# DeepMed-Lab-ECNU/BCP

Hardware: AMD Instinct MI355X
Metric: training volumes/sec (LA 112x112x80 V-Net, BCP self-training step) (higher is better)
Workload: dtype f32 (fp16x2 split operands); 1 GPU; LA 3D V-Net BCP self-train step, per-GPU batch 4 (2 labeled), 112x112x80 patches, SGD m0.9 wd1e-4, EMA 0.99 (BASELINE.json configs[1]); global_batch=4, parallelism=dp1

## Files before the change

### bcp_amd/csrc/api.hip

```cpp
#include "common.h"
#include "../../include/bcp_hip.h"
#include <cstring>

namespace bcp {
static thread_local char g_err[512] = "";
void set_error(const char* fmt, ...) {
  va_list ap;
  va_start(ap, fmt);
  vsnprintf(g_err, sizeof(g_err), fmt, ap);
  va_end(ap);
}
Options& options() {
  static Options o;
  return o;
}
}

extern "C" int bcp_version(void) { return BCP_ABI_VERSION; }

extern "C" int bcp_set_option(const char* name, const char* value) {
  BCP_REQUIRE(name && value, "bcp_set_option: null argument");
  bcp::Options& o = bcp::options();
  const bcp::Options def;
  long long v[5] = {0, 0, 0, 0, 0};
  const int n = sscanf(value, "%lld,%lld,%lld,%lld,%lld", &v[0], &v[1], &v[2], &v[3], &v[4]);
  const bool reset = n <= 0;
#define BCP_OPT_INT(field) if (!strcmp(name, #field)) { o.field = reset ? def.field : (int)v[0]; return BCP_OK; }
  BCP_OPT_INT(conv3_p) BCP_OPT_INT(splitk) BCP_OPT_INT(conv3_b6_flat_sk) BCP_OPT_INT(conv3_b6_cfg2d) BCP_OPT_INT(conv3_b6_w22) BCP_OPT_INT(conv3_b6_pipe) BCP_OPT_INT(conv3_b6_cin16max) BCP_OPT_INT(res_pcu) BCP_OPT_INT(res_nt) BCP_OPT_INT(wgrad_nt)
  BCP_OPT_INT(tn_groups) BCP_OPT_INT(cc_tile) BCP_OPT_INT(pack_sections) BCP_OPT_INT(cc_select_blocks) BCP_OPT_INT(conv3_b6) BCP_OPT_INT(conv3_b6_levels) BCP_OPT_INT(conv3_b6_direct) BCP_OPT_INT(conv3_b6_flat) BCP_OPT_INT(conv3_b6_minvox) BCP_OPT_INT(wgrad_b6) BCP_OPT_INT(wgrad_b6_minvox) BCP_OPT_INT(wgrad_b6_levels) BCP_OPT_INT(wgrad_b6_slots) BCP_OPT_INT(cc_border_dedupe) BCP_OPT_INT(cc_count_tile) BCP_OPT_INT(cc_fuse_select) BCP_OPT_INT(gemm_walk) BCP_OPT_INT(gemm_pipe) BCP_OPT_INT(gemm_stat_r) BCP_OPT_INT(norm_apply_cap) BCP_OPT_INT(norm_apply_vec) BCP_OPT_INT(k2_stats) BCP_OPT_INT(k2_bwd_stats) BCP_OPT_INT(up_recompute) BCP_OPT_INT(wgrad_b6_deep) BCP_OPT_INT(wgrad_b6_deep_nt) BCP_OPT_INT(wgrad_b6_deep_slots) BCP_OPT_INT(wgrad_b6_deep_tile) BCP_OPT_INT(norm_slabs) BCP_OPT_INT(conv3_f16) BCP_OPT_INT(fuse_bwd_stats) BCP_OPT_INT(conv3_xcd) BCP_OPT_INT(mix_c1) BCP_OPT_INT(whatif) BCP_OPT_INT(c3d16_form) BCP_OPT_INT(norm_own) BCP_OPT_INT(wgrad_reduce_flat) BCP_OPT_INT(norm_fin_rows) BCP_OPT_INT(norm_fuse_fin)
#undef BCP_OPT_INT
  if (!strcmp(name, "conv3_sk_elems")) { o.conv3_sk_elems = reset ? def.conv3_sk_elems : v[0]; return BCP_OK; }
  if (!strcmp(name, "res_tile2d_vox")) { o.res_tile2d_vox = reset ? def.res_tile2d_vox : v[0]; return BCP_OK; }
  if (!strcmp(name, "conv3_cfg")) {
    BCP_REQUIRE(reset || n == 4, "bcp_set_option: conv3_cfg wants TD,TH,TW,NT");
    for (int i = 0; i < 4; ++i) o.conv3_cfg[i] = reset ? 0 : (int)v[i];
    return BCP_OK;
  }
  if (!strcmp(name, "wgrad_tile")) {
    BCP_REQUIRE(reset || n >= 3, "bcp_set_option: wgrad_tile wants TD,TH,TW[,min_voxels,max_voxels]");
    for (int i = 0; i < 5; ++i) o.wgrad_tile[i] = def.wgrad_tile[i];
    for (int i = 0; i < n && !reset; ++i) o.wgrad_tile[i] = v[i];
    return BCP_OK;
  }
  bcp::set_error("bcp_set_option: unknown option '%s'", name);
  return BCP_EINVAL;
}
extern "C" const char* bcp_last_error(void) { return bcp::g_err; }

extern "C" int bcp_device_arch(char* buf, int n) {
  BCP_REQUIRE(buf && n > 0, "bcp_device_arch: bad buffer");
  int dev = 0;
  hipDeviceProp_t prop;
  if (hipGetDevice(&dev) != hipSuccess || hipGetDeviceProperties(&prop, dev) != hipSuccess) {
    bcp::set_error("bcp_device_arch: no HIP device");
    return BCP_ELAUNCH;
  }
  strncpy(buf, prop.gcnArchName, (size_t)n - 1);
  buf[n - 1] = 0;
  return BCP_OK;
}

extern "C" int bcp_event_create(void** ev) {
  BCP_REQUIRE(ev, "bcp_event_create: null");
  hipEvent_t e;
  if (hipEventCreate(&e) != hipSuccess) { bcp::set_error("hipEventCreate failed"); return BCP_ELAUNCH; }
  *ev = (void*)e;
  return BCP_OK;
}
extern "C" int bcp_event_record(void* ev, void* stream) {
  if (hipEventRecord((hipEvent_t)ev, (hipStream_t)stream) != hipSuccess) { bcp::set_error("hipEventRecord failed"); return BCP_ELAUNCH; }
  return BCP_OK;
}
extern "C" int bcp_event_elapsed_ms(void* start, void* stop, float* ms) {
  BCP_REQUIRE(ms, "bcp_event_elapsed_ms: null");
  if (hipEventSynchronize((hipEvent_t)stop) != hipSuccess || hipEventElapsedTime(ms, (hipEvent_t)start, (hipEvent_t)stop) != hipSuccess) {
    bcp::set_error("hipEventElapsedTime failed");
    return BCP_ELAUNCH;
  }
  return BCP_OK;
}
extern "C" int bcp_event_destroy(void* ev) {
  hipEventDestroy((hipEvent_t)ev);
// ... 36 lines not shown
```

### bcp_amd/csrc/common.h

```cpp
#pragma once
#include <hip/hip_runtime.h>
#include <cstdarg>
#include <cstdint>
#include <cstdio>

#define BCP_OK 0
#define BCP_EINVAL (-1)
#define BCP_ELAUNCH (-2)
#define BCP_EUNSUP (-3)

typedef float f32x4 __attribute__((ext_vector_type(4)));

namespace bcp {

void set_error(const char* fmt, ...);

#define BCP_REQUIRE(cond, ...)          \
  do {                                  \
    if (!(cond)) {                      \
      ::bcp::set_error(__VA_ARGS__);    \
      return BCP_EINVAL;                \
    }                                   \
  } while (0)

// ... 8 lines not shown

struct Options {
  int conv3_p = 0;
  int splitk = 0;
  long long conv3_sk_elems = 1LL << 20;
  int conv3_b6_cin16max = 32;
  int conv3_b6_pipe = 1;
  int conv3_b6_w22 = 1;
  int conv3_b6_cfg2d = 1;
  int conv3_b6_flat_sk = 0;
  int res_pcu = 0;
  int res_nt = 0;
  long long res_tile2d_vox = 10000;
  int conv3_cfg[4] = {0, 0, 0, 0};
  int wgrad_nt = 0;
  long long wgrad_tile[5] = {0, 0, 0, 0, 1LL << 60};
  int tn_groups = 0;
  int pack_sections = 7;
  int cc_tile = 0;
  int cc_select_blocks = 0;
  int conv3_b6 = 1;
  int conv3_b6_levels = 15;
  int conv3_b6_minvox = 256;
  int conv3_b6_flat = 1;
  int conv3_b6_direct = 1;
  int wgrad_b6 = 1;
  int wgrad_b6_minvox = 256;
  int norm_slabs = 1;
  int fuse_bwd_stats = 1;
  int conv3_xcd = 11;
  int conv3_f16 = 1;
  int wgrad_b6_slots = 0;
  int mix_c1 = 1;
  int wgrad_b6_deep = 1;
  int wgrad_b6_deep_nt = 0;
  int wgrad_b6_deep_slots = 0;
  int wgrad_b6_deep_tile = 1;
  int k2_stats = 2;
  int up_recompute = 0;
  int k2_bwd_stats = 0;
  int norm_fuse_fin = 1;
  int norm_fin_rows = 128;
  int gemm_pipe = 1;
  int gemm_stat_r = 0;
  int gemm_walk = 0;
  int cc_border_dedupe = 1;
  int cc_count_tile = 0;
  int cc_fuse_select = 1;
  int norm_apply_cap = 2048;
  int norm_apply_vec = 4;
  int wgrad_reduce_flat = 1;
  int norm_own = 0;
  int c3d16_form = 1;
  int whatif = 0;
  int wgrad_b6_levels = 15;
};
Options& options();

__device__ __forceinline__ unsigned char plabel_bin_of(float x0, float x1, float thres) {
  const float m = fmaxf(x0, x1);
  const float e0 = expf(x0 - m), e1 = expf(x1 - m);
  const float p1 = e1 / (e0 + e1);
  return (p1 >= thres) ? 1 : 0;
}
__device__ __forceinline__ unsigned char plabel_argmax4_of(float x0, float x1, float x2, float x3) {
  const float m = fmaxf(fmaxf(x0, x1), fmaxf(x2, x3));
  const float e0 = expf(x0 - m), e1 = expf(x1 - m), e2 = expf(x2 - m), e3 = expf(x3 - m);
  const float s = e0 + e1 + e2 + e3;
  const float p0 = e0 / s, p1 = e1 / s, p2 = e2 / s, p3 = e3 / s;
  int best = 0;
  float pb = p0;
  if (p1 > pb) { pb = p1; best = 1; }
  if (p2 > pb) { pb = p2; best = 2; }
  if (p3 > pb) { pb = p3; best = 3; }
  return (unsigned char)best;
}


static inline int cdiv(long long a, long long b) { return (int)((a + b - 1) / b); }
static inline bool aligned16(const void* p) { return (reinterpret_cast<uintptr_t>(p) & 15u) == 0; }

#ifndef BCP_LDS_BARRIER
#define BCP_LDS_BARRIER() asm volatile("s_waitcnt lgkmcnt(0)\n\ts_barrier" ::: "memory")
#endif

#ifndef BCP_GLDS16
typedef __attribute__((address_space(3))) void* bcp_lds_ptr_t;
#define BCP_GLDS16(gsrc, lds_wave_base) __builtin_amdgcn_global_load_lds((gsrc), (bcp_lds_ptr_t)(lds_wave_base), 16, 0, 0)
#define BCP_VM_LDS_BARRIER(N) asm volatile("s_waitcnt vmcnt(%0) lgkmcnt(0)\n\ts_barrier" ::"n"(N) : "memory")
#endif

#ifndef BCP_S_SLEEP
#define BCP_S_SLEEP(n) __builtin_amdgcn_s_sleep(n)
#endif

__device__ __forceinline__ float wave_sum(float v) {
#pragma unroll
  for (int o = 32; o > 0; o >>= 1) v += __shfl_xor(v, o);
  return v;
}
__device__ __forceinline__ double wave_sum(double v) {
#pragma unroll
  for (int o = 32; o > 0; o >>= 1) v += __shfl_xor(v, o);
  return v;
}

__device__ __forceinline__ unsigned long long wave_sum(unsigned long long v) {
#pragma unroll
  for (int o = 32; o > 0; o >>= 1) v += __shfl_xor(v, o);
  return v;
}

template <int NV>
__device__ __forceinline__ void block_sum_256(double (&v)[NV], double* lds ) {
  const int lane = threadIdx.x & 63, wid = threadIdx.x >> 6;
#pragma unroll
  for (int i = 0; i < NV; ++i) v[i] = wave_sum(v[i]);
  __syncthreads();
  if (lane == 0) {
#pragma unroll
    for (int i = 0; i < NV; ++i) lds[wid * NV + i] = v[i];
  }
  __syncthreads();
  if (threadIdx.x == 0) {
#pragma unroll
    for (int i = 0; i < NV; ++i) v[i] = lds[i] + lds[NV + i] + lds[2 * NV + i] + lds[3 * NV + i];
  }
}

constexpr int kAmaxSlots = 32, kAmaxStride = 32, kAmaxFloats = kAmaxSlots * kAmaxStride;
__device__ __forceinline__ void amax_clear(float* __restrict__ slots) {
  if (threadIdx.x < kAmaxSlots) slots[threadIdx.x * kAmaxStride] = 0.f;
}
__device__ __forceinline__ void block_amax_publish(float m, float* __restrict__ slots) {
  __shared__ float amax_red[4];
#pragma unroll
  for (int o = 32; o > 0; o >>= 1) { const float t = __shfl_xor(m, o); m = (t > m || t != t) ? t : m; }
  if ((threadIdx.x & 63) == 0) amax_red[threadIdx.x >> 6] = m;
// ... 46 lines not shown
```

### bcp_amd/csrc/conv3.hip

```cpp
#include "conv3_defs.h"
#include "../../include/bcp_hip.h"
#include <cstdlib>
#include <cstdio>

namespace bcp {

template <int KD, int TD, int TH, int TW, int NT, int WT>
__global__ __launch_bounds__(256) void k_conv3_mfma(const float* __restrict__ X, const float* __restrict__ Wp,
                                                    const float* __restrict__ bias, float* __restrict__ Y, ConvDims cd,
                                                    int accumulate, StatsArg st) {
  using TL = Tile<KD, TD, TH, TW>;
  constexpr int MT = TL::MT, T = TL::T, CT = NT * 16;
  constexpr int S = T / WT;
  static_assert(T % WT == 0, "WT must divide the tap count");
  constexpr int NBUF = (S > 1) ? 2 : 1;
  constexpr int WSTAGE4 = WT * 4 * CT;
  constexpr int NW4 = (WSTAGE4 + 255) / 256;
  constexpr int NACC = (MT * NT == 1) ? 2 : 1;

  HIP_DYNAMIC_SHARED(float4, smem4)
  float* smem = reinterpret_cast<float*>(smem4);
  float* Xs = smem;
  float* Ws = smem + TL::HV * XS;
  double* Ss = reinterpret_cast<double*>(Ws + NBUF * WSTAGE4 * 4);

  const int lane = threadIdx.x & 63, wave = threadIdx.x >> 6;
  const int li = lane & 15, lg = lane >> 4;
  int n, d0, h0, w0;
  tile_origin(cd, blockIdx.x, TD, TH, TW, n, d0, h0, w0);
  const int cout0 = blockIdx.y * CT;
  const int cin4 = cd.Cin16 >> 2;

  int voff[MT];
#pragma unroll
  for (int mt = 0; mt < MT; ++mt) voff[mt] = TL::voff((wave * MT + mt) * 16 + li) * XS + lg * 4;
  HaloFetch<TL> hf;
  hf.init(cd, Xs);

  f32x4 acc[NACC][MT][NT];
#pragma unroll
  for (int a = 0; a < NACC; ++a)
#pragma unroll
    for (int mt = 0; mt < MT; ++mt)
#pragma unroll
      for (int nt = 0; nt < NT; ++nt) acc[a][mt][nt] = (f32x4){0.f, 0.f, 0.f, 0.f};

  const int nchunks = cd.Cin16 >> 4;
  const int c_begin = (int)((long long)nchunks * blockIdx.z / gridDim.z), c_end = (int)((long long)nchunks * (blockIdx.z + 1) / gridDim.z);
  Y += (long long)blockIdx.z * cd.N * cd.D * cd.H * cd.W * cd.Cout;
  if (S == 1) {
    float4 hpre[HaloFetch<TL>::NP], wpre[NW4];
    auto wfetch = [&](int cc) {
#pragma unroll
      for (int u = 0; u < NW4; ++u) {
        const int q = threadIdx.x + u * 256;
// ... 917 lines not shown
      uchar4 m4 = make_uchar4(1, 1, 1, 1);
      if (EPI >= 3 && ok) dav = ld4(nm.da + e);
      if (has_mask && ok) m4 = nm.mask_seed ? bern_keep4(e, mseed_lo, mseed_hi, nm.p_keep) : *reinterpret_cast<const uchar4*>(nm.elem_mask + e);
      f32x4 acc = (f32x4){0.f, 0.f, 0.f, 0.f};
#pragma unroll
      for (int ks = 0; ks < KS; ++ks) acc = __builtin_amdgcn_mfma_f32_16x16x4f32(wv[ks], Xs[vo + toff[ks]], acc, 0, 0, 0);
      float4 dyl = make_float4(0.f, 0.f, 0.f, 0.f);
      if (ok) {
        const float yv[4] = {acc[0] + bv.x, acc[1] + bv.y, acc[2] + bv.z, acc[3] + bv.w};
        if (EPI == 0) st4(Y + e, make_float4(yv[0], yv[1], yv[2], yv[3]));
        if (EPI <= 1) {
          if (st.partial) {
#pragma unroll
            for (int r = 0; r < 4; ++r) { s1[r] += (double)yv[r]; s2[r] += (double)yv[r] * (double)yv[r]; }
          }
        } else {
          const float ms[4] = {m4.x ? nm.elem_scale : 0.f, m4.y ? nm.elem_scale : 0.f, m4.z ? nm.elem_scale : 0.f, m4.w ? nm.elem_scale : 0.f};
          const float dd[4] = {dav.x, dav.y, dav.z, dav.w};
          float o[4];
#pragma unroll
          for (int r = 0; r < 4; ++r) {
            const float z = (yv[r] - mu[r]) * sc[r] + sh[r];
            if (EPI == 2) {
              o[r] = act_fwd(z, nm.act);
              if (has_mask) o[r] *= ms[r];
              const float t = fabsf(o[r]);
              amax_o = (t > amax_o || t != t) ? t : amax_o;
            } else {
              const float cs = has_mask ? ms[r] : 1.f;
              const float dz = dd[r] * cs * act_grad(z, nm.act);
              const float xh = (yv[r] - mu[r]) * rs[r];
              if (EPI == 3) { s1[r] += (double)dz; s2[r] += (double)dz * (double)xh; }
              else o[r] = sc[r] * (dz - k1[r] - xh * k2[r]);
            }
          }
          if (EPI == 2 || EPI == 4) st4(Y + e, make_float4(o[0], o[1], o[2], o[3]));
          if (EPI == 5) dyl = make_float4(o[0], o[1], o[2], o[3]);
        }
      }
      if (EPI == 5) st4(Ys + m * 16 + lg * 4, dyl);
    }
    if (EPI == 5) {
      __syncthreads();
#pragma unroll 4
      for (int ks = 0; ks < 16; ++ks) {
        const int v = wave * 64 + ks * 4 + lg;
        const int vo = TL::voff(v);
        const float b = Ys[v * 16 + li];
        wacc[0] = __builtin_amdgcn_mfma_f32_16x16x4f32(Xs[vo + aoff[0]], b, wacc[0], 0, 0, 0);
        wacc[1] = __builtin_amdgcn_mfma_f32_16x16x4f32(Xs[vo + aoff[1]], b, wacc[1], 0, 0, 0);
      }
    }
  }
  if (EPI == 5) {
    __syncthreads();
    float* red = Ys;
#pragma unroll
    for (int tt = 0; tt < 2; ++tt)
#pragma unroll
      for (int r = 0; r < 4; ++r) red[(wave * 32 + tt * 16 + lg * 4 + r) * 16 + li] = wacc[tt][r];
    __syncthreads();
    for (int o = threadIdx.x; o < T * 16; o += 256)
      Y[(long long)blockIdx.x * T * 16 + o] = (red[o] + red[512 + o]) + (red[1024 + o] + red[1536 + o]);
  }
  if (st.partial) {
#pragma unroll
    for (int r = 0; r < 4; ++r) {
      double a = s1[r], b = s2[r];
#pragma unroll
      for (int o = 1; o < 16; o <<= 1) { a += __shfl_xor(a, o); b += __shfl_xor(b, o); }
      if (li == 0) { Ss[(wave * 16 + lg * 4 + r) * 2] = a; Ss[(wave * 16 + lg * 4 + r) * 2 + 1] = b; }
    }
    __syncthreads();
    if (threadIdx.x < 16) {
      const int c = threadIdx.x;
      double a = 0.0, b = 0.0;
#pragma unroll
      for (int wv_ = 0; wv_ < 4; ++wv_) { a += Ss[(wv_ * 16 + c) * 2]; b += Ss[(wv_ * 16 + c) * 2 + 1]; }
      const int gg = t_begin / st.tiles_per_group, row = (t_begin % st.tiles_per_group) / tiles_per_block;
      double* dst = st.partial + (((long long)gg * st.rows + row) * 16 + c) * 2;
      dst[0] = a; dst[1] = b;
    }
  }
  if (EPI == 2 && nm.amax) { __syncthreads(); block_amax_publish(amax_o, nm.amax); }
}

template <int KD, int TD, int TH, int TW>
__global__ __launch_bounds__(256) void k_conv3_c1_wgrad(const float* __restrict__ X, const float* __restrict__ dY,
                                                        float* __restrict__ partial, ConvDims cd, int tiles_total,
                                                        int tiles_per_group) {
  using TL = Tile<KD, TD, TH, TW>;
  constexpr int T = TL::T, M = TL::M;
  static_assert(M == 256 && T <= 32, "four waves x 64 voxels, two 16-tap MFMA row tiles");
  constexpr int NXS = (TL::HV + 255) / 256;
  __shared__ __attribute__((aligned(16))) float Xs[TL::HV];
  __shared__ __attribute__((aligned(16))) float Ys[M * 16];
  const int lane = threadIdx.x & 63, wave = threadIdx.x >> 6;
  const int li = lane & 15, lg = lane >> 4;
  const int grp = blockIdx.x;
  int t_end = (grp + 1) * tiles_per_group;
  if (t_end > tiles_total) t_end = tiles_total;
  int tile = grp * tiles_per_group;
  if (tile >= t_end) return;

  int aoff[2];
#pragma unroll
// ... 484 lines not shown
  const Cfg c = choose_wgrad_cfg(KD, N, D, H, W, Co16);
  const int g = wgrad_groups(c, N, D, H, W, Ci16, Co16);
  const size_t a = (size_t)g * KD * 9 * Ci16 * Co16 * sizeof(float), c6 = b6_wgrad_workspace_bytes(cd, KD);
  return a > c6 ? a : c6;
}

#define BCP_WG_CASE(KD_, TD_, TH_, TW_, NT_)                                                     \
  if (c.KD == KD_ && c.TD == TD_ && c.TH == TH_ && c.TW == TW_ && c.NT == NT_) {                 \
    G = launch_wgrad<KD_, TD_, TH_, TW_, NT_>(x, dy, ws, cd, groups, (hipStream_t)stream);       \
    done = true;                                                                                 \
  }

extern "C" int bcp_conv3_wgrad(const float* x, const float* dy, float* dw, int N, int D, int H, int W, int Cin, int Cout, int KD,
                               int accumulate, void* workspace, const float* x_amax_or_null, const float* dy_amax_or_null, void* stream) {
  if (bcp::options().whatif & 8) return BCP_OK;

  BCP_REQUIRE(x && dy && dw && workspace, "bcp_conv3_wgrad: null pointer");
  BCP_REQUIRE((KD == 1 || KD == 3) && N > 0 && D > 0 && H > 0 && W > 0, "bcp_conv3_wgrad: bad extents");
  BCP_REQUIRE(Cin % 4 == 0 && Cout % 4 == 0, "bcp_conv3_wgrad: Cin/Cout must be multiples of 4");
  ConvDims cd;
  fill_dims(cd, N, D, H, W, Cin, Cout);
  bool done = false;
  const Cfg c = choose_wgrad_cfg(KD, N, D, H, W, cd.Cout16);
  const int groups = wgrad_groups(c, N, D, H, W, cd.Cin16, cd.Cout16);
  float* ws = reinterpret_cast<float*>(workspace);
  if (x_amax_or_null && dy_amax_or_null) { cd.xamax = x_amax_or_null; cd.yamax = dy_amax_or_null; }
  int G = b6_wgrad(x, dy, ws, dw, accumulate, cd, KD, (hipStream_t)stream);
  if (G < 0) {
    BCP_CHECK_LAUNCH("bcp_conv3_wgrad");
    return BCP_OK;
  }
  if (G > 0) done = true;
  if (!done) {
  BCP_WG_CASE(3, 4, 4, 16, 1) BCP_WG_CASE(3, 4, 4, 16, 2) BCP_WG_CASE(3, 4, 4, 16, 4)
  BCP_WG_CASE(3, 4, 8, 8, 1) BCP_WG_CASE(3, 4, 8, 8, 2) BCP_WG_CASE(3, 4, 8, 8, 4)
  BCP_WG_CASE(3, 4, 4, 8, 1) BCP_WG_CASE(3, 4, 4, 8, 2) BCP_WG_CASE(3, 4, 4, 8, 4)
  BCP_WG_CASE(3, 4, 4, 4, 1) BCP_WG_CASE(3, 4, 4, 4, 2) BCP_WG_CASE(3, 4, 4, 4, 4)
  BCP_WG_CASE(3, 2, 8, 4, 1) BCP_WG_CASE(3, 2, 8, 4, 2) BCP_WG_CASE(3, 2, 8, 4, 4)
  BCP_WG_CASE(1, 1, 16, 16, 1) BCP_WG_CASE(1, 1, 16, 16, 2) BCP_WG_CASE(1, 1, 16, 16, 4)
  BCP_WG_CASE(1, 1, 8, 8, 1) BCP_WG_CASE(1, 1, 8, 8, 2) BCP_WG_CASE(1, 1, 8, 8, 4)
  }
  BCP_REQUIRE(done, "bcp_conv3_wgrad: no kernel instance for KD=%d tile=%dx%dx%d NT=%d", c.KD, c.TD, c.TH, c.TW, c.NT);
  const int T = KD * 9;
  if (G >= 32 || options().wgrad_reduce_flat == 2)
    launch_reduce_deep(ws, dw, G, T, Cin, Cout, cd.Cin16, cd.Cout16, accumulate, (hipStream_t)stream);
  else
    hipLaunchKernelGGL(k_wgrad_reduce, dim3(Cin, cdiv(Cout, 64)), dim3(256), 0, (hipStream_t)stream, ws, dw, G, T, Cin, Cout, cd.Cin16,
                       cd.Cout16, accumulate);
  BCP_CHECK_LAUNCH("bcp_conv3_wgrad");
  return BCP_OK;
}

static int c1_tiles_per_block(int tiles_per_group) {
  for (int t = 8; t > 1; t >>= 1)
    if (tiles_per_group % t == 0 && tiles_per_group / t >= 256) return t;
  return 1;
}

template <int EPI>
static void c1_launch(int KD, dim3 grid, hipStream_t s, const float* x, const float* w, const float* bias, float* y, const ConvDims& cd, int tiles,
                      int tpb, const StatsArg& st, const C1Norm& nm) {
  if (KD == 3) hipLaunchKernelGGL((k_conv3_c1<3, 4, 4, 16, EPI>), grid, dim3(256), 0, s, x, w, bias, y, cd, tiles, tpb, st, nm);
  else hipLaunchKernelGGL((k_conv3_c1<1, 1, 16, 16, EPI>), grid, dim3(256), 0, s, x, w, bias, y, cd, tiles, tpb, st, nm);
}

static int c1_fwd_impl(const float* x, const float* w, const float* bias, float* y, int N, int D, int H, int W, int KD, double* stat_partial,
                       int groups, bool dry, hipStream_t s, int epi = 0, const C1Norm* nmp = nullptr) {
  ConvDims cd;
  fill_dims(cd, N, D, H, W, 1, 16);
  if (KD == 3) { cd.tiles_d = cdiv(D, 4); cd.tiles_h = cdiv(H, 4); cd.tiles_w = cdiv(W, 16); }
  else { cd.tiles_d = 1; cd.tiles_h = cdiv(H, 16); cd.tiles_w = cdiv(W, 16); }
  const int tiles = N * cd.tiles_d * cd.tiles_h * cd.tiles_w;
  StatsArg st{nullptr, 0, 1, 16, groups > 0 ? groups : 1};
  int tpb = 1;
  if (groups > 0) {
    if (N % groups) return 0;
    const int tpg = tiles / groups;
    tpb = c1_tiles_per_block(tpg);
    st.tiles_per_group = tpg; st.rows = tpg / tpb; st.partial = stat_partial;
    if (dry) return st.rows;
  }
  const dim3 grid(cdiv(tiles, tpb));
  const C1Norm none{nullptr, nullptr, nullptr, nullptr, 1.f, 0, 1, nullptr};
  const C1Norm& nm = nmp ? *nmp : none;
  switch (epi) {
    case 1: c1_launch<1>(KD, grid, s, x, w, bias, y, cd, tiles, tpb, st, nm); break;
    case 2: c1_launch<2>(KD, grid, s, x, w, bias, y, cd, tiles, tpb, st, nm); break;
    case 3: c1_launch<3>(KD, grid, s, x, w, bias, y, cd, tiles, tpb, st, nm); break;
    case 4: c1_launch<4>(KD, grid, s, x, w, bias, y, cd, tiles, tpb, st, nm); break;
    case 5: c1_launch<5>(KD, grid, s, x, w, bias, y, cd, tiles, tpb, st, nm); break;
    default: c1_launch<0>(KD, grid, s, x, w, bias, y, cd, tiles, tpb, st, nm); break;
  }
  return st.rows;
}

extern "C" int bcp_conv3_c1_fwd(const float* x, const float* w, const float* bias, float* y, int N, int D, int H, int W, int KD,
                                void* stream) {
  BCP_REQUIRE(x && w && y, "bcp_conv3_c1_fwd: null pointer");
  BCP_REQUIRE((KD == 1 && D == 1) || KD == 3, "bcp_conv3_c1_fwd: bad KD/D");
  BCP_REQUIRE(aligned16(y) && (!bias || aligned16(bias)), "bcp_conv3_c1_fwd: y / bias must be 16-B aligned");
  c1_fwd_impl(x, w, bias, y, N, D, H, W, KD, nullptr, 0, false, (hipStream_t)stream);
  BCP_CHECK_LAUNCH("bcp_conv3_c1_fwd");
  return BCP_OK;
}

extern "C" int bcp_conv3_c1_stat_rows(int N, int D, int H, int W, int KD, int groups) {
  if (groups < 1 || N < 1 || D < 1 || H < 1 || W < 1 || !((KD == 1 && D == 1) || KD == 3)) return 0;
  return c1_fwd_impl(nullptr, nullptr, nullptr, nullptr, N, D, H, W, KD, nullptr, groups, true, nullptr);
}

extern "C" int bcp_conv3_c1_fwd_stats(const float* x, const float* w, const float* bias, float* y, int N, int D, int H, int W, int KD,
                                      double* stat_partial, int groups, void* stream) {
  BCP_REQUIRE(x && w && y && stat_partial && groups >= 1, "bcp_conv3_c1_fwd_stats: null pointer / bad groups");
  BCP_REQUIRE((KD == 1 && D == 1) || KD == 3, "bcp_conv3_c1_fwd_stats: bad KD/D");
  BCP_REQUIRE(aligned16(y) && (!bias || aligned16(bias)), "bcp_conv3_c1_fwd_stats: y / bias must be 16-B aligned");
  const int rows = c1_fwd_impl(x, w, bias, y, N, D, H, W, KD, stat_partial, groups, false, (hipStream_t)stream);
  BCP_REQUIRE(rows > 0, "bcp_conv3_c1_fwd_stats: fused statistics unavailable (N %% groups != 0): check bcp_conv3_c1_stat_rows first");
  BCP_CHECK_LAUNCH("bcp_conv3_c1_fwd_stats");
  return BCP_OK;
}

namespace bcp {
void norm_fwd_finalize_launch(const double* partial, int nb, int G, int C, long long rows_per_group, const float* gamma, const float* beta,
                              float* running_mean, float* running_var, float momentum, float eps, float* stats, hipStream_t s, float* amax_clear_or_null);
void norm_bwd_finalize_launch(const double* partial, int nb, int G, int C, long long rows_per_group, float* dgamma, float* dbeta, int accumulate,
                              float* c1c2raw, hipStream_t s, float* amax_clear_or_null);
}

extern "C" size_t bcp_conv3_c1_norm_workspace_bytes(int N, int D, int H, int W, int KD, int groups) {
  const int rows = bcp_conv3_c1_stat_rows(N, D, H, W, KD, groups);
  return rows > 0 ? (size_t)groups * rows * 16 * 2 * sizeof(double) + (size_t)4 * groups * 16 * sizeof(float) : 0;
}

// ... 103 lines not shown
```

Baseline: 825.0 volumes/s.

## Add streamlined single-input-channel conv kernel with prefetched halo and packed tap offsets

Adds a new k_conv3_c1s kernel for the Cin=1 convolution and selects it by default for KD=3 through the c1_form option. It prefetches the next tile's halo into registers while the MFMAs run on the current one, using double-buffered LDS. Tap offsets are packed into registers and bounds checks are done with one-hot masks. A compile-time all-full variant drops per-tile bounds checks and requests higher occupancy, and sched_group_barrier hints interleave LDS reads with MFMAs. This adds code size and register pressure and depends on correct halo masking at borders; a c1_tpb override is also added.

```diff
diff --git a/bcp_amd/csrc/api.hip b/bcp_amd/csrc/api.hip
--- a/bcp_amd/csrc/api.hip
+++ b/bcp_amd/csrc/api.hip
@@ -27,7 +27,7 @@
   const bool reset = n <= 0;
 #define BCP_OPT_INT(field) if (!strcmp(name, #field)) { o.field = reset ? def.field : (int)v[0]; return BCP_OK; }
   BCP_OPT_INT(conv3_p) BCP_OPT_INT(splitk) BCP_OPT_INT(conv3_b6_flat_sk) BCP_OPT_INT(conv3_b6_cfg2d) BCP_OPT_INT(conv3_b6_w22) BCP_OPT_INT(conv3_b6_pipe) BCP_OPT_INT(conv3_b6_cin16max) BCP_OPT_INT(res_pcu) BCP_OPT_INT(res_nt) BCP_OPT_INT(wgrad_nt)
-  BCP_OPT_INT(tn_groups) BCP_OPT_INT(cc_tile) BCP_OPT_INT(pack_sections) BCP_OPT_INT(cc_select_blocks) BCP_OPT_INT(conv3_b6) BCP_OPT_INT(conv3_b6_levels) BCP_OPT_INT(conv3_b6_direct) BCP_OPT_INT(conv3_b6_flat) BCP_OPT_INT(conv3_b6_minvox) BCP_OPT_INT(wgrad_b6) BCP_OPT_INT(wgrad_b6_minvox) BCP_OPT_INT(wgrad_b6_levels) BCP_OPT_INT(wgrad_b6_slots) BCP_OPT_INT(cc_border_dedupe) BCP_OPT_INT(cc_count_tile) BCP_OPT_INT(cc_fuse_select) BCP_OPT_INT(gemm_walk) BCP_OPT_INT(gemm_pipe) BCP_OPT_INT(gemm_stat_r) BCP_OPT_INT(norm_apply_cap) BCP_OPT_INT(norm_apply_vec) BCP_OPT_INT(k2_stats) BCP_OPT_INT(k2_bwd_stats) BCP_OPT_INT(up_recompute) BCP_OPT_INT(wgrad_b6_deep) BCP_OPT_INT(wgrad_b6_deep_nt) BCP_OPT_INT(wgrad_b6_deep_slots) BCP_OPT_INT(wgrad_b6_deep_tile) BCP_OPT_INT(norm_slabs) BCP_OPT_INT(conv3_f16) BCP_OPT_INT(fuse_bwd_stats) BCP_OPT_INT(conv3_xcd) BCP_OPT_INT(mix_c1) BCP_OPT_INT(whatif) BCP_OPT_INT(c3d16_form) BCP_OPT_INT(norm_own) BCP_OPT_INT(wgrad_reduce_flat) BCP_OPT_INT(norm_fin_rows) BCP_OPT_INT(norm_fuse_fin)
+  BCP_OPT_INT(tn_groups) BCP_OPT_INT(cc_tile) BCP_OPT_INT(pack_sections) BCP_OPT_INT(cc_select_blocks) BCP_OPT_INT(conv3_b6) BCP_OPT_INT(conv3_b6_levels) BCP_OPT_INT(conv3_b6_direct) BCP_OPT_INT(conv3_b6_flat) BCP_OPT_INT(conv3_b6_minvox) BCP_OPT_INT(wgrad_b6) BCP_OPT_INT(wgrad_b6_minvox) BCP_OPT_INT(wgrad_b6_levels) BCP_OPT_INT(wgrad_b6_slots) BCP_OPT_INT(cc_border_dedupe) BCP_OPT_INT(cc_count_tile) BCP_OPT_INT(cc_fuse_select) BCP_OPT_INT(gemm_walk) BCP_OPT_INT(gemm_pipe) BCP_OPT_INT(gemm_stat_r) BCP_OPT_INT(norm_apply_cap) BCP_OPT_INT(norm_apply_vec) BCP_OPT_INT(k2_stats) BCP_OPT_INT(k2_bwd_stats) BCP_OPT_INT(up_recompute) BCP_OPT_INT(wgrad_b6_deep) BCP_OPT_INT(wgrad_b6_deep_nt) BCP_OPT_INT(wgrad_b6_deep_slots) BCP_OPT_INT(wgrad_b6_deep_tile) BCP_OPT_INT(norm_slabs) BCP_OPT_INT(conv3_f16) BCP_OPT_INT(fuse_bwd_stats) BCP_OPT_INT(conv3_xcd) BCP_OPT_INT(mix_c1) BCP_OPT_INT(whatif) BCP_OPT_INT(c3d16_form) BCP_OPT_INT(c1_form) BCP_OPT_INT(c1_tpb) BCP_OPT_INT(norm_own) BCP_OPT_INT(wgrad_reduce_flat) BCP_OPT_INT(norm_fin_rows) BCP_OPT_INT(norm_fuse_fin)
 #undef BCP_OPT_INT
   if (!strcmp(name, "conv3_sk_elems")) { o.conv3_sk_elems = reset ? def.conv3_sk_elems : v[0]; return BCP_OK; }
   if (!strcmp(name, "res_tile2d_vox")) { o.res_tile2d_vox = reset ? def.res_tile2d_vox : v[0]; return BCP_OK; }
diff --git a/bcp_amd/csrc/common.h b/bcp_amd/csrc/common.h
--- a/bcp_amd/csrc/common.h
+++ b/bcp_amd/csrc/common.h
@@ -84,6 +84,8 @@
   int wgrad_reduce_flat = 1;
   int norm_own = 0;
   int c3d16_form = 1;
+  int c1_form = 1;
+  int c1_tpb = 0;
   int whatif = 0;
   int wgrad_b6_levels = 15;
 };
@@ -116,6 +118,18 @@
 #define BCP_LDS_BARRIER() asm volatile("s_waitcnt lgkmcnt(0)\n\ts_barrier" ::: "memory")
 #endif
 
+#ifndef BCP_SETTLE
+#define BCP_SETTLE(x) asm volatile("" : "+v"(x))
+#endif
+
+#ifndef BCP_GLOBAL
+#define BCP_GLOBAL __attribute__((address_space(1)))
+#endif
+
+#ifndef BCP_SCHED_GROUP
+#define BCP_SCHED_GROUP(mask, n) __builtin_amdgcn_sched_group_barrier((mask), (n), 0)
+#endif
+
 #ifndef BCP_GLDS16
 typedef __attribute__((address_space(3))) void* bcp_lds_ptr_t;
 #define BCP_GLDS16(gsrc, lds_wave_base) __builtin_amdgcn_global_load_lds((gsrc), (bcp_lds_ptr_t)(lds_wave_base), 16, 0, 0)
diff --git a/bcp_amd/csrc/conv3.hip b/bcp_amd/csrc/conv3.hip
--- a/bcp_amd/csrc/conv3.hip
+++ b/bcp_amd/csrc/conv3.hip
@@ -1,6 +1,7 @@
 #include "conv3_defs.h"
 #include "../../include/bcp_hip.h"
 #include <cstdlib>
+#include <type_traits>
 #include <cstdio>
 
 namespace bcp {
@@ -1024,6 +1025,346 @@
       }
     }
   }
+  if (EPI == 5) {
+    __syncthreads();
+    float* red = Ys;
+#pragma unroll
+    for (int tt = 0; tt < 2; ++tt)
+#pragma unroll
+      for (int r = 0; r < 4; ++r) red[(wave * 32 + tt * 16 + lg * 4 + r) * 16 + li] = wacc[tt][r];
+    __syncthreads();
+    for (int o = threadIdx.x; o < T * 16; o += 256)
+      Y[(long long)blockIdx.x * T * 16 + o] = (red[o] + red[512 + o]) + (red[1024 + o] + red[1536 + o]);
+  }
+  if (st.partial) {
+#pragma unroll
+    for (int r = 0; r < 4; ++r) {
+      double a = s1[r], b = s2[r];
+#pragma unroll
+      for (int o = 1; o < 16; o <<= 1) { a += __shfl_xor(a, o); b += __shfl_xor(b, o); }
+      if (li == 0) { Ss[(wave * 16 + lg * 4 + r) * 2] = a; Ss[(wave * 16 + lg * 4 + r) * 2 + 1] = b; }
+    }
+    __syncthreads();
+    if (threadIdx.x < 16) {
+      const int c = threadIdx.x;
+      double a = 0.0, b = 0.0;
+#pragma unroll
+      for (int wv_ = 0; wv_ < 4; ++wv_) { a += Ss[(wv_ * 16 + c) * 2]; b += Ss[(wv_ * 16 + c) * 2 + 1]; }
+      const int gg = t_begin / st.tiles_per_group, row = (t_begin % st.tiles_per_group) / tiles_per_block;
+      double* dst = st.partial + (((long long)gg * st.rows + row) * 16 + c) * 2;
+      dst[0] = a; dst[1] = b;
+    }
+  }
+  if (EPI == 2 && nm.amax) { __syncthreads(); block_amax_publish(amax_o, nm.amax); }
+}
+
+template <bool B> struct C1Flag { static constexpr bool value = B; };
+
+template <int KD, int TD, int TH, int TW, int EPI, bool ALL_FULL>
+__global__ __launch_bounds__(256, ALL_FULL ? 4 : 2) void k_conv3_c1s(const float* __restrict__ X, const float* __restrict__ w ,
+                                                                      const float* __restrict__ bias, float* __restrict__ Y, ConvDims cd,
+                                                                      int n_tiles, int tiles_per_block, StatsArg st, C1Norm nm) {
+  constexpr bool all_full = ALL_FULL;
+  using TL = Tile<KD, TD, TH, TW>;
+  constexpr int T = TL::T, MT = TL::MT, KS = (T + 3) / 4;
+  constexpr int HVA = (TL::HV + 3) & ~3;
+  constexpr int AHEAD = KS < 2 ? KS : 2;
+  static_assert(TW == 16 && MT == 4 && TL::M == 256 && TH % MT == 0,
+                "a wave's m-tile is one 16-voxel w line: m = (wave * 4 + mt) * 16 + li, and its four lines are consecutive h");
+  __shared__ __attribute__((aligned(16))) float Xs[2 * HVA];
+  __shared__ float Ws[KS * 64];
+  __shared__ __attribute__((aligned(16))) float Cs[4 * 7 * 4];
+  __shared__ double Ss[4 * 16 * 2];
+  __shared__ __attribute__((aligned(16))) float Ys[EPI == 5 ? TL::M * 16 : 4];
+  static_assert(EPI != 5 || T <= 32, "EPI 5: two 16-tap MFMA row tiles");
+  const int lane = threadIdx.x & 63, wave = threadIdx.x >> 6;
+  const int li = lane & 15, lg = lane >> 4;
+  static_assert(TL::HV <= 1024, "packed tap offsets");
+  unsigned aq = 0;
+  f32x4 wacc[2] = {(f32x4){0.f, 0.f, 0.f, 0.f}, (f32x4){0.f, 0.f, 0.f, 0.f}};
+  if (EPI == 5) {
+#pragma unroll
+    for (int tt = 0; tt < 2; ++tt) aq |= (unsigned)((tt * 16 + li < T) ? TL::tapoff(tt * 16 + li) : 0) << (16 * tt);
+  }
+  unsigned tq[(KS + 2) / 3];
+#pragma unroll
+  for (int j = 0; j < (KS + 2) / 3; ++j) tq[j] = 0;
+#pragma unroll
+  for (int ks = 0; ks < KS; ++ks) {
+    const int tap = ks * 4 + lg;
+    tq[ks / 3] |= (unsigned)(tap < T ? TL::tapoff(tap) : 0) << (10 * (ks % 3));
+    if (wave == 0) Ws[ks * 64 + lane] = tap < T ? w[li * T + tap] : 0.f;
+  }
+  double s1[4] = {0, 0, 0, 0}, s2[4] = {0, 0, 0, 0};
+  float amax_o = 0.f;
+  unsigned mseed_lo = 0, mseed_hi = 0;
+  if (EPI >= 2 && nm.mask_seed) { const unsigned long long s_ = *nm.mask_seed; mseed_lo = (unsigned)s_; mseed_hi = (unsigned)(s_ >> 32); }
+  const bool has_mask = EPI >= 2 && (nm.elem_mask != nullptr || nm.mask_seed != nullptr);
+  const bool a_relu = nm.act == ACT_RELU, a_lrelu = nm.act == ACT_LRELU;
+  const float g_neg = a_lrelu ? 0.01f : (a_relu ? 0.f : 1.f);
+  auto actf = [&](float z) __attribute__((always_inline)) -> float { const float neg = a_lrelu ? 0.01f * z : (a_relu ? 0.f : z); return z > 0.f ? z : neg; };
+  auto actg = [&](float z) __attribute__((always_inline)) -> float { return z > 0.f ? 1.f : g_neg; };
+  const bool mask_ld = EPI >= 2 && nm.elem_mask != nullptr && nm.mask_seed == nullptr;
+  const int t_begin = blockIdx.x * tiles_per_block;
+  int t_end = t_begin + tiles_per_block;
+  if (t_end > n_tiles) t_end = n_tiles;
+  if (wave == 0 && li == 0) {
+    float* c = Cs + lg * 28;
+    st4(c, bias ? ld4(bias + lg * 4) : make_float4(0.f, 0.f, 0.f, 0.f));
+    if (EPI >= 2) {
+      const int g = t_begin / st.tiles_per_group;
+      const long long GC = (long long)nm.G * 16, o = (long long)g * 16 + lg * 4;
+#pragma unroll
+      for (int r = 0; r < 4; ++r) {
+        c[4 + r] = nm.stats[o + r]; c[8 + r] = nm.stats[GC + o + r]; c[12 + r] = nm.stats[2 * GC + o + r]; c[16 + r] = nm.stats[3 * GC + o + r];
+        if (EPI >= 4) { c[20 + r] = nm.c1c2[o + r]; c[24 + r] = nm.c1c2[GC + o + r]; }
+      }
+    }
+  }
+  int tn, ttd, tth, ttw;
+  {
+    int d0, h0, w0;
+    tile_origin(cd, t_begin, TD, TH, TW, tn, d0, h0, w0);
+    tn = __builtin_amdgcn_readfirstlane(tn); ttd = __builtin_amdgcn_readfirstlane(d0 / TD);
+    tth = __builtin_amdgcn_readfirstlane(h0 / TH); ttw = __builtin_amdgcn_readfirstlane(w0 / TW);
+  }
+  auto step = [&]() __attribute__((always_inline)) {
+    ttw += 1;
+    const int cw = ttw == cd.tiles_w ? 1 : 0;
+    ttw = cw ? 0 : ttw; tth += cw;
+    const int ch = tth == cd.tiles_h ? 1 : 0;
+    tth = ch ? 0 : tth; ttd += ch;
+    const int cdd = ttd == cd.tiles_d ? 1 : 0;
+    ttd = cdd ? 0 : ttd; tn += cdd;
+  };
+  constexpr int NPRE = (TL::HV + 255) / 256;
+  constexpr int HB_D = TL::PD ? TL::HD : 0, HBITS = HB_D + TL::HH + TL::HW;
+  static_assert(HBITS <= 64, "one-hot halo coordinates");
+  using hmask_t = typename std::conditional<(HBITS <= 32), unsigned, unsigned long long>::type;
+  float pre[NPRE];
+  unsigned pre_in = 0;
+  unsigned hrel[NPRE];
+  hmask_t hbit[NPRE];
+#pragma unroll
+  for (int i = 0; i < NPRE; ++i) {
+    int q = threadIdx.x + i * 256;
+    if (q > TL::HV - 1) q = TL::HV - 1;
+    const int hw = q % TL::HW, hh = (q / TL::HW) % TL::HH, hd = q / (TL::HW * TL::HH);
+    hrel[i] = (unsigned)((hd * cd.H + hh) * cd.W + hw) * 4u;
+    hbit[i] = ((hmask_t)1 << (HB_D + hh)) | ((hmask_t)1 << (HB_D + TL::HH + hw)) | (TL::PD ? ((hmask_t)1 << hd) : (hmask_t)0);
+  }
+  const unsigned crel = (unsigned)((TL::PD * cd.H + 1) * cd.W + 1) * 4u;
+  auto ival = [](int lo, int hi) __attribute__((always_inline)) -> hmask_t {
+    return (((hmask_t)1 << hi) - 1) & ~(((hmask_t)1 << lo) - 1);
+  };
+  auto fetch = [&](int n, int d0, int h0, int w0) __attribute__((always_inline)) {
+    const long long corner = (((long long)n * cd.D + (d0 - TL::PD)) * cd.H + (h0 - 1)) * cd.W + (w0 - 1);
+    const char* xc = reinterpret_cast<const char*>(X + corner);
+    const int dlo = TL::PD - d0 > 0 ? TL::PD - d0 : 0, dhi = cd.D - d0 + TL::PD < TL::HD ? cd.D - d0 + TL::PD : TL::HD;
+    const int hlo = 1 - h0 > 0 ? 1 - h0 : 0, hhi = cd.H - h0 + 1 < TL::HH ? cd.H - h0 + 1 : TL::HH;
+    const int wlo = 1 - w0 > 0 ? 1 - w0 : 0, whi = cd.W - w0 + 1 < TL::HW ? cd.W - w0 + 1 : TL::HW;
+    const hmask_t tm = (TL::PD ? ival(dlo, dhi) : (hmask_t)0) | (ival(hlo, hhi) << HB_D) | (ival(wlo, whi) << (HB_D + TL::HH));
+    pre_in = 0;
+#pragma unroll
+    for (int i = 0; i < NPRE; ++i) {
+      const bool in = (hbit[i] & tm) == hbit[i];
+      pre_in |= in ? 1u << i : 0u;
+      pre[i] = *reinterpret_cast<const float*>(xc + (in ? hrel[i] : crel));
+    }
+  };
+  auto stash = [&](float* xs) __attribute__((always_inline)) {
+#pragma unroll
+    for (int i = 0; i < NPRE; ++i)
+      if (threadIdx.x + i * 256 < TL::HV) xs[threadIdx.x + i * 256] = ((pre_in >> i) & 1u) ? pre[i] : 0.f;
+  };
+  const int q0 = wave * MT;
+  const unsigned lane_el = ((unsigned)((q0 / TH) * cd.H + q0 % TH) * (unsigned)cd.W + li) * 16u + lg * 4;
+  const unsigned lane_b = lane_el * 4u;
+  const long long mt_el = (long long)cd.W * 16;
+  auto tile_base = [&](int n, int d0, int h0, int w0) __attribute__((always_inline)) -> long long {
+    return ((((long long)n * cd.D + d0) * cd.H + h0) * cd.W + w0) * 16;
+  };
+  auto inside = [&](int d0, int h0, int w0, int mt) __attribute__((always_inline)) -> bool {
+    return d0 + q0 / TH < cd.D && h0 + q0 % TH + mt < cd.H && w0 + li < cd.W;
+  };
+  auto ld4b = [](const float* p, unsigned b) __attribute__((always_inline)) -> float4 {
+    return *reinterpret_cast<const float4*>(reinterpret_cast<const char*>(p) + b);
+  };
+  float4 dav[MT];
+#pragma unroll
+  for (int mt = 0; mt < MT; ++mt) dav[mt] = make_float4(0.f, 0.f, 0.f, 0.f);
+
+  int cn = tn, cd0 = ttd * TD, ch0 = tth * TH, cw0 = ttw * TW;
+  fetch(cn, cd0, ch0, cw0);
+  if (EPI >= 3) {
+    const int d0 = cd0, h0 = ch0, w0 = cw0;
+    const long long tb = tile_base(cn, cd0, ch0, cw0);
+#pragma unroll
+    for (int mt = 0; mt < MT; ++mt)
+      if (all_full || inside(d0, h0, w0, mt)) dav[mt] = ld4b(nm.da + tb + mt * mt_el, lane_b);
+  }
+  stash(Xs);
+  BCP_LDS_BARRIER();
+
+  auto body = [&](int tile, auto next_c, auto full_c) __attribute__((always_inline)) {
+    constexpr bool NEXT = decltype(next_c)::value, FULL = decltype(full_c)::value;
+    const float* xs = Xs + ((tile - t_begin) & 1) * HVA;
+    const int d0 = cd0, h0 = ch0, w0 = cw0;
+    const long long tb = tile_base(cn, d0, h0, w0);
+    const bool full = FULL || (d0 + TD <= cd.D && h0 + TH <= cd.H && w0 + TW <= cd.W);
+    bool ok[MT];
+#pragma unroll
+    for (int mt = 0; mt < MT; ++mt) ok[mt] = full || inside(d0, h0, w0, mt);
+    unsigned m4[MT];
+#pragma unroll
+    for (int mt = 0; mt < MT; ++mt) m4[mt] = 0x01010101u;
+    int n2 = 0, d2 = 0, h2 = 0, w2 = 0;
+    long long tb2 = 0;
+    if (NEXT) {
+      step();
+      n2 = tn; d2 = ttd * TD; h2 = tth * TH; w2 = ttw * TW;
+      fetch(n2, d2, h2, w2);
+      tb2 = tile_base(n2, d2, h2, w2);
+    }
+    __builtin_amdgcn_sched_barrier(0);
+    float xb[MT][KS], wv[KS];
+    int toff[KS];
+#pragma unroll
+    for (int j = 0; j < (KS + 2) / 3; ++j) {
+      unsigned t = tq[j];
+      BCP_SETTLE(t);
+#pragma unroll
+      for (int ks = 3 * j; ks < 3 * j + 3 && ks < KS; ++ks) toff[ks] = (int)((t >> (10 * (ks % 3))) & 0x3ffu);
+    }
+    const int vo0 = TL::voff(q0 * 16 + li);
+    f32x4 acc[MT];
+#pragma unroll
+    for (int mt = 0; mt < MT; ++mt) acc[mt] = (f32x4){0.f, 0.f, 0.f, 0.f};
+#pragma unroll
+    for (int ks = 0; ks < AHEAD; ++ks) {
+      wv[ks] = Ws[ks * 64 + lane];
+#pragma unroll
+      for (int mt = 0; mt < MT; ++mt) xb[mt][ks] = xs[vo0 + mt * TL::HW + toff[ks]];
+    }
+#pragma unroll
+    for (int ks = 0; ks < KS; ++ks) {
+      if (ks + AHEAD < KS) {
+        wv[ks + AHEAD] = Ws[(ks + AHEAD) * 64 + lane];
+#pragma unroll
+        for (int mt = 0; mt < MT; ++mt) xb[mt][ks + AHEAD] = xs[vo0 + mt * TL::HW + toff[ks + AHEAD]];
+      }
+#pragma unroll
+      for (int mt = 0; mt < MT; ++mt) acc[mt] = __builtin_amdgcn_mfma_f32_16x16x4f32(wv[ks], xb[mt][ks], acc[mt], 0, 0, 0);
+    }
+    BCP_SCHED_GROUP(0x100, (MT + 1) * AHEAD);
+#pragma unroll
+    for (int ks = 0; ks < KS; ++ks) {
+      if (ks + AHEAD < KS) BCP_SCHED_GROUP(0x100, MT + 1);
+      BCP_SCHED_GROUP(0x008, MT);
+    }
+    __builtin_amdgcn_sched_barrier(0);
+    if (mask_ld) {
+#pragma unroll
+      for (int mt = 0; mt < MT; ++mt)
+        if (ok[mt]) m4[mt] = *(const BCP_GLOBAL unsigned*)(nm.elem_mask + tb + mt * mt_el + lane_el);
+#pragma unroll
+      for (int mt = 0; mt < MT; ++mt) BCP_SETTLE(m4[mt]);
+    }
+    const float4 bv = ld4(Cs + lg * 28);
+    float mu[4] = {0, 0, 0, 0}, rs[4] = {1, 1, 1, 1}, sc[4] = {1, 1, 1, 1}, sh[4] = {0, 0, 0, 0}, k1[4] = {0, 0, 0, 0}, k2[4] = {0, 0, 0, 0};
+    if (EPI >= 2) {
+      const float4 a = ld4(Cs + lg * 28 + 4), b = ld4(Cs + lg * 28 + 8), c = ld4(Cs + lg * 28 + 12), d = ld4(Cs + lg * 28 + 16);
+      mu[0] = a.x; mu[1] = a.y; mu[2] = a.z; mu[3] = a.w;
+      rs[0] = b.x; rs[1] = b.y; rs[2] = b.z; rs[3] = b.w;
+      sc[0] = c.x; sc[1] = c.y; sc[2] = c.z; sc[3] = c.w;
+      sh[0] = d.x; sh[1] = d.y; sh[2] = d.z; sh[3] = d.w;
+      if (EPI >= 4) {
+        const float4 f = ld4(Cs + lg * 28 + 20), g = ld4(Cs + lg * 28 + 24);
+        k1[0] = f.x; k1[1] = f.y; k1[2] = f.z; k1[3] = f.w;
+        k2[0] = g.x; k2[1] = g.y; k2[2] = g.z; k2[3] = g.w;
+      }
+    }
+#pragma unroll
+    for (int mt = 0; mt < MT; ++mt) {
+      const int m = (q0 + mt) * 16 + li;
+      float* yp = reinterpret_cast<float*>(reinterpret_cast<char*>(Y + tb + mt * mt_el) + lane_b);
+      float4 dyl = make_float4(0.f, 0.f, 0.f, 0.f);
+      if (ok[mt]) {
+        const f32x4 a4 = acc[mt];
+        const float yv[4] = {a4[0] + bv.x, a4[1] + bv.y, a4[2] + bv.z, a4[3] + bv.w};
+        if (EPI == 0) st4(yp, make_float4(yv[0], yv[1], yv[2], yv[3]));
+        if (EPI <= 1) {
+          if (st.partial) {
+#pragma unroll
+            for (int r = 0; r < 4; ++r) { s1[r] += (double)yv[r]; s2[r] += (double)yv[r] * (double)yv[r]; }
+          }
+        } else {
+          unsigned mk = m4[mt];
+          if (EPI >= 2 && nm.mask_seed) {
+            unsigned le = lane_el;
+            BCP_SETTLE(le);
+            const uchar4 k4 = bern_keep4(tb + mt * mt_el + le, mseed_lo, mseed_hi, nm.p_keep);
+            mk = k4.x | (k4.y << 8) | (k4.z << 16) | ((unsigned)k4.w << 24);
+          }
+          const float ms[4] = {(mk & 0xffu) ? nm.elem_scale : 0.f, (mk & 0xff00u) ? nm.elem_scale : 0.f, (mk & 0xff0000u) ? nm.elem_scale : 0.f,
+                               (mk & 0xff000000u) ? nm.elem_scale : 0.f};
+          const float dd[4] = {dav[mt].x, dav[mt].y, dav[mt].z, dav[mt].w};
+          float o[4];
+#pragma unroll
+          for (int r = 0; r < 4; ++r) {
+            const float z = (yv[r] - mu[r]) * sc[r] + sh[r];
+            if (EPI == 2) {
+              o[r] = actf(z);
+              if (has_mask) o[r] *= ms[r];
+              const float t = fabsf(o[r]);
+              amax_o = (t > amax_o || t != t) ? t : amax_o;
+            } else {
+              const float cs = has_mask ? ms[r] : 1.f;
+              const float dz = dd[r] * cs * actg(z);
+              const float xh = (yv[r] - mu[r]) * rs[r];
+              if (EPI == 3) { s1[r] += (double)dz; s2[r] += (double)dz * (double)xh; }
+              else o[r] = sc[r] * (dz - k1[r] - xh * k2[r]);
+            }
+          }
+          if (EPI == 2 || EPI == 4) st4(yp, make_float4(o[0], o[1], o[2], o[3]));
+          if (EPI == 5) dyl = make_float4(o[0], o[1], o[2], o[3]);
+        }
+      }
+      if (EPI == 5) st4(Ys + m * 16 + lg * 4, dyl);
+      if (EPI == 1 || EPI == 3) {
+#pragma unroll
+        for (int r = 0; r < 4; ++r) { BCP_SETTLE(s1[r]); BCP_SETTLE(s2[r]); }
+      }
+      if (EPI >= 3 && NEXT) {
+        __builtin_amdgcn_sched_barrier(0);
+        dav[mt] = make_float4(0.f, 0.f, 0.f, 0.f);
+        if (FULL || inside(d2, h2, w2, mt)) dav[mt] = ld4b(nm.da + tb2 + mt * mt_el, lane_b);
+      }
+      __builtin_amdgcn_sched_barrier(0);
+    }
+    if (EPI == 5) {
+      BCP_LDS_BARRIER();
+      unsigned aqv = aq;
+      BCP_SETTLE(aqv);
+      const int aoff[2] = {(int)(aqv & 0xffffu), (int)(aqv >> 16)};
+#pragma unroll 4
+      for (int ks = 0; ks < 16; ++ks) {
+        const int v = wave * 64 + ks * 4 + lg;
+        const int vo = TL::voff(v);
+        const float b = Ys[v * 16 + li];
+        wacc[0] = __builtin_amdgcn_mfma_f32_16x16x4f32(xs[vo + aoff[0]], b, wacc[0], 0, 0, 0);
+        wacc[1] = __builtin_amdgcn_mfma_f32_16x16x4f32(xs[vo + aoff[1]], b, wacc[1], 0, 0, 0);
+      }
+    }
+    if (NEXT) {
+      stash(Xs + (((tile - t_begin) & 1) ^ 1) * HVA);
+      BCP_LDS_BARRIER();
+      cn = n2; cd0 = d2; ch0 = h2; cw0 = w2;
+    }
+  };
+  for (int tile = t_begin; tile < t_end - 1; ++tile) body(tile, C1Flag<true>(), C1Flag<ALL_FULL>());
+  body(t_end - 1, C1Flag<false>(), C1Flag<ALL_FULL>());
+
   if (EPI == 5) {
     __syncthreads();
     float* red = Ys;
@@ -1614,6 +1955,8 @@
 }
 
 static int c1_tiles_per_block(int tiles_per_group) {
+  const int forced = options().c1_tpb;
+  if (forced > 0 && tiles_per_group % forced == 0) return forced;
   for (int t = 8; t > 1; t >>= 1)
     if (tiles_per_group % t == 0 && tiles_per_group / t >= 256) return t;
   return 1;
@@ -1622,6 +1965,15 @@
 template <int EPI>
 static void c1_launch(int KD, dim3 grid, hipStream_t s, const float* x, const float* w, const float* bias, float* y, const ConvDims& cd, int tiles,
                       int tpb, const StatsArg& st, const C1Norm& nm) {
+  const int form = options().c1_form;
+  if ((form == 2 || (form == 1 && KD == 3)) && 4LL * cd.H * cd.W < (1LL << 26) && (long long)cd.D * cd.H * cd.W < (1LL << 30)) {
+    const bool all_full = KD == 3 ? (cd.D % 4 == 0 && cd.H % 4 == 0 && cd.W % 16 == 0) : (cd.H % 16 == 0 && cd.W % 16 == 0);
+    if (KD == 3 && all_full) hipLaunchKernelGGL((k_conv3_c1s<3, 4, 4, 16, EPI, true>), grid, dim3(256), 0, s, x, w, bias, y, cd, tiles, tpb, st, nm);
+    else if (KD == 3) hipLaunchKernelGGL((k_conv3_c1s<3, 4, 4, 16, EPI, false>), grid, dim3(256), 0, s, x, w, bias, y, cd, tiles, tpb, st, nm);
+    else if (all_full) hipLaunchKernelGGL((k_conv3_c1s<1, 1, 16, 16, EPI, true>), grid, dim3(256), 0, s, x, w, bias, y, cd, tiles, tpb, st, nm);
+    else hipLaunchKernelGGL((k_conv3_c1s<1, 1, 16, 16, EPI, false>), grid, dim3(256), 0, s, x, w, bias, y, cd, tiles, tpb, st, nm);
+    return;
+  }
   if (KD == 3) hipLaunchKernelGGL((k_conv3_c1<3, 4, 4, 16, EPI>), grid, dim3(256), 0, s, x, w, bias, y, cd, tiles, tpb, st, nm);
   else hipLaunchKernelGGL((k_conv3_c1<1, 1, 16, 16, EPI>), grid, dim3(256), 0, s, x, w, bias, y, cd, tiles, tpb, st, nm);
 }
@@ -1641,6 +1993,8 @@
     tpb = c1_tiles_per_block(tpg);
     st.tiles_per_group = tpg; st.rows = tpg / tpb; st.partial = stat_partial;
     if (dry) return st.rows;
+  } else if (options().c1_tpb > 0 && tiles % options().c1_tpb == 0) {
+    tpb = options().c1_tpb;
   }
   const dim3 grid(cdiv(tiles, tpb));
   const C1Norm none{nullptr, nullptr, nullptr, nullptr, 1.f, 0, 1, nullptr};
```

Result: no change. 829.0 volumes/s (median of 6 runs) (+0.5%).
